# bioinf/Sibelia

Hardware: AMD Instinct MI355X
Metric: k-mers/sec in BlockFinder graph-build+simplify, 8xE.coli k=25 (higher is better)
Workload: dtype u64; 1 GPU; 8 synthetic E. coli-like strains x 4.6 Mbp (gen_strains seed 1, 1% SNP, indels, inversions), k=25 D=150 maxIterations=4, one full stage; strand_kmers_per_gpu=73598388, parallelism=1 GPU, exchange_bytes_rank0=0, bulges=334284, bif_ids=1120044, instances=7089276, rounds=106, replays=0, device_bytes=22762263122

## Files before the change

sibelia_amd/csrc/rounds.hip:

```cpp
#include <cstring>
#include <algorithm>
#include <vector>
#include "simplify_walks.h"

__device__ __forceinline__ int wave_probe_window(const GraphView &g, const ScanBurst &raw, unsigned dir, unsigned ws, VerdictTable &vt, unsigned lane,
                                                 unsigned id, unsigned tid, unsigned &distinct)
{
	ScanView b;
	burst_view(g, raw, dir, ws, lane, 3u, b);
	const unsigned k = g.k, D = g.D;
	if (k >= 64u * SCAN_BURST) return -2;
	unsigned firstbad = ~0u, firstsep = ~0u;
#pragma unroll
	for (int u = 0; u < SCAN_BURST; u++) {
		const unsigned long long in = __ballot(b.inr[u]), good = __ballot(b.inr[u] && b.plink[u] == b.cc[u]), sep = __ballot(b.inr[u] && b.chv[u] == BT_SEP);
		const unsigned long long bad = in & ~good;
		if (bad && firstbad == ~0u) firstbad = 64u * u + (unsigned)__builtin_ctzll(bad);
		if (sep && firstsep == ~0u) firstsep = 64u * u + (unsigned)__builtin_ctzll(sep);
	}
	const unsigned covered = ws < 64u * SCAN_BURST ? ws : 64u * SCAN_BURST;
	const unsigned len = firstsep < covered ? firstsep : covered;
	if (firstbad < len || firstbad <= firstsep && firstbad < covered) return -2;
	if (firstsep >= covered && covered < ws && D > covered) return -2;
	bool viol = false;
// ... 300 lines not shown
			const unsigned long long todo = __ballot(act && slow && j == 0u);
			if (pass == 1) {
				if (act && !slow) ecmask |= bit;
				for (unsigned long long td = todo; td; td &= td - 1ull) {
					const unsigned src = (unsigned)__builtin_ctzll(td);
					const unsigned wa = __shfl(a, src), wd = __shfl(dir, src);
					const WalkedWindow ww = idx_walk_window(g, wa, wd, k + 1u, lane, id, tid, nullptr, nullptr, 0u);
					if (ww.viol) viol = true;
					if (ww.len >= k + 1u) { const char e2 = wd ? bt_comp((char)ww.craw) : (char)ww.craw; ecmask |= e2 == 'A' ? 1u : e2 == 'C' ? 2u : e2 == 'G' ? 4u : 8u; }
				}
				continue;
			}
			const unsigned own = act ? s_own[i] : 0u;
			const unsigned lim = len < D ? len : D, upper = own < lim ? own : lim;
			unsigned long long cm = act && !slow && bit ? mk & vm & idx_bits(1 - t0, (int)upper - t0) : 0ull;
			unsigned total = (unsigned)__popcll(cm);
			for (int d = 32; d > 0; d >>= 1) total += __shfl_xor(total, d);
			const bool tight = distinct + total > VT_FILL;
			const unsigned *__restrict__ marks = g.bif[dir];
			while (__any(cm != 0ull)) {
				if (tight) {
					unsigned nins = (unsigned)__popcll(cm);
					nins = nins < 4u ? nins : 4u;
					for (int d = 32; d > 0; d >>= 1) nins += __shfl_xor(nins, d);
					if (distinct + nins > VT_HARD) return -1;
				}
				unsigned sl[4]; bool has[4]; unsigned bb[4];
#pragma unroll
				for (int q = 0; q < 4; q++) {
					has[q] = cm != 0ull;
					const unsigned r = has[q] ? (unsigned)__builtin_ctzll(cm) : 0u;
					if (has[q]) cm &= cm - 1ull;
					const unsigned step = (unsigned)(t0 + (int)r);
					sl[q] = has[q] ? (dir ? a - step : a + step) : a;
				}
#pragma unroll
				for (int q = 0; q < 4; q++) bb[q] = marks[fresh ? 0u : sl[q]];
				bool found = false;
#pragma unroll
				for (int q = 0; q < 4; q++) found |= vt_insert(vt, has[q] ? bb[q] : BT_NONE, bit, distinct);
				if (found) { if (viol) wave_stamp(g, 0, tid, 3, id, 0, tid + 1); return 1; }
			}
			for (unsigned long long td = todo; td; td &= td - 1ull) {
				const unsigned src = (unsigned)__builtin_ctzll(td);
				const unsigned wa = __shfl(a, src), wd = __shfl(dir, src);
				WSYNC();
				const WalkedWindow ww = idx_walk_window(g, wa, wd, ws, lane, id, tid, mk_step, mk_id, walk_marks);
				if (ww.viol) viol = true;
				if (ww.overflow) return -1;
				WSYNC();
				if (ww.len < k + 1u) continue;
				const char e2 = wd ? bt_comp((char)ww.craw) : (char)ww.craw;
				const unsigned b2 = e2 == 'A' ? 1u : e2 == 'C' ? 2u : e2 == 'G' ? 4u : 8u;
				const unsigned lim2 = ww.len < D ? ww.len : D;
				bool found = false;
				for (unsigned m0 = 0; m0 < ww.nm; m0 += 64) {
					if (distinct + (ww.nm - m0 < 64u ? ww.nm - m0 : 64u) > VT_HARD) return -1;
					const unsigned m = m0 + lane;
					const bool ok = m < ww.nm && mk_step[m] < lim2;
					found |= vt_insert(vt, ok ? mk_id[m] : BT_NONE, b2, distinct);
				}
				if (found) { if (viol) wave_stamp(g, 0, tid, 3, id, 0, tid + 1); return 1; }
			}
		}
		if (pass == 1) {
			for (int d = 32; d > 0; d >>= 1) ecmask |= __shfl_xor(ecmask, d);
			if (__popc(ecmask) <= 1) { if (viol) wave_stamp(g, 0, tid, 3, id, 0, tid + 1); return 0; }
		}
	}
	if (viol) wave_stamp(g, 0, tid, 3, id, 0, tid + 1);
	return 0;
}
__global__ void __launch_bounds__(64) k_probe_idx(GraphView g, unsigned nwin, uint8_t *live, unsigned w0, unsigned vbits, unsigned max_inst, unsigned walk_marks,
                                                  unsigned *__restrict__ instbuf, unsigned istride, int snapshot)
{
	extern __shared__ unsigned pidx_dyn[];
	VtRef vt; vt.key = pidx_dyn; vt.mask = pidx_dyn + (1u << vbits); vt.bits = vbits;
	unsigned *const s_sel = vt.mask + (1u << vbits), *const s_own = s_sel + max_inst, *const s_mkstep = s_own + max_inst, *const s_mkid = s_mkstep + walk_marks;
	uint8_t *const s_dir = reinterpret_cast<uint8_t *>(s_mkid + walk_marks);
	const unsigned wi = blockIdx.x + w0, lane = threadIdx.x;
	if (!snapshot) round_stamp(g, 0);
	if (wi >= nwin) return;
	const unsigned id = g.win[wi], tid = snapshot ? 0xFFFFFFFEu : id + 1;
	const bool known_live = !snapshot && g.need[id] == 2;
	if (known_live && !(instbuf && bt_parked(g, id))) { if (lane == 0) { live[wi] = 1; if (instbuf) instbuf[(size_t)wi * istride] = BT_NONE; if (g.test_flags & BT_TF_STATS) atomicAdd(&g_idx_stats[0], 1u); } return; }
	const unsigned n = wave_list_nodes(g, g.head[0][id], g.head[1][id], lane, nullptr, [&](unsigned off, unsigned, unsigned s, unsigned el, unsigned) {
		if (off < max_inst) { s_sel[off] = el; s_dir[off] = (uint8_t)s; }
	});
	int r = 0;
	if (known_live) {
		if (lane == 0) live[wi] = 1;
		unsigned *ib = instbuf + (size_t)wi * istride;
		const bool give = n <= max_inst && n + 1u <= istride;
		if (give) { WSYNC(); for (unsigned i = lane; i < n; i += 64) ib[1 + i] = (s_sel[i] << 1) | s_dir[i]; }
		if (lane == 0) ib[0] = give ? n : BT_NONE;
		return;
	}
	if (n >= 2) {
		if (n > max_inst || (!g.any_parked && n != g.lsize[0][id] + g.lsize[1][id])) r = -1;
		else { WSYNC(); r = probe_idx(g, vt, s_sel, s_dir, s_own, s_mkstep, s_mkid, walk_marks, n, lane, id, tid); }
	}
	if (lane == 0) {
		if (r < 0) live[wi] = PROBE_UNSERVED;
		else if (r == 0) { g.need[id] = 0; g.touch[id] = 0; live[wi] = 0; }
		else { g.need[id] = 2; live[wi] = 1; }
		if (g.test_flags & BT_TF_STATS) atomicAdd(&g_idx_stats[n < 2 ? 1 : r == 0 ? 2 : r == 1 ? 3 : r == -1 ? 4 : 5], 1u);
	}
	if (instbuf) {
		unsigned *ib = instbuf + (size_t)wi * istride;
		const bool give = r == 1 && n + 1u <= istride;
		if (give) { WSYNC(); for (unsigned i = lane; i < n; i += 64) ib[1 + i] = (s_sel[i] << 1) | s_dir[i]; }
		if (lane == 0) ib[0] = give ? n : BT_NONE;
	}
}

static_assert(PROBE_WAVES == 1u, "k_probe synchronises its lanes with WSYNC(): one wave per workgroup");
__global__ void __launch_bounds__(64 * PROBE_WAVES) k_probe(GraphView g, unsigned nwin, uint8_t *arena, unsigned arena_bytes, uint8_t *live, unsigned w0, int snapshot)
{
	__shared__ Txn t;
	__shared__ BulgeWork w;
	__shared__ VerdictTable vt;
	__shared__ int ok;
	__shared__ __attribute__((aligned(16))) uint8_t fast[2048];
	const unsigned wi = blockIdx.x + w0, lane = threadIdx.x & 63u;
	if (!g.idx_probe && !snapshot) round_stamp(g, 0);
	if (wi >= nwin) return;
	if ((g.idx_probe || snapshot) && live[wi] != PROBE_UNSERVED) return;
	const unsigned id = g.win[wi], tid = snapshot ? 0xFFFFFFFEu : id + 1;
	if (!snapshot && g.need[id] == 2) { if (threadIdx.x == 0) live[wi] = 1; return; }
	if (threadIdx.x == 0) { t.init(g, id, wi, snapshot ? 0u : 3u, arena + (size_t)(!snapshot && g.slice_busy && g.slice_busy[wi] ? g.shadow_base + wi : wi) * arena_bytes, arena_bytes); t.ext_stamps = true; t.fscr = fast; t.fscr_cap = sizeof fast; }
	WSYNC();
	wave_setup<true>(g, t, w, true, lane, ok);
	for (unsigned i = threadIdx.x; i < VT_SLOTS; i += 64 * PROBE_WAVES) { vt.key[i] = BT_NONE; vt.mask[i] = 0; }
	WSYNC();
	int verdict = 0;
	if (ok && probe_endchars(g, w, lane, id, tid)) ok = 0;
	if (ok) {
		verdict = probe_windows(g, w, vt, lane, id, tid);
		if (verdict < 0) {
			for (unsigned i = 0; i < w.n; i++) wave_scan_instance(g, w, i, lane, 0, tid, 3, id);
			WSYNC();
		}
	}
	if (lane == 0) {
		bool has = verdict > 0;
		if (verdict < 0) { bt_end_chars(t, w); has = bt_any_bulges(t, w, true); }
		if (t.err) has = true;
		if (!has) { g.need[id] = 0; g.touch[id] = 0; }
		else if (!t.err) g.need[id] = 2;
		else if (snapshot) g.need[id] = 1;
		live[wi] = has ? (t.err ? 2 : 1) : 0;
	}
}
__global__ void __launch_bounds__(256) k_pack_need(const unsigned *__restrict__ perm, const uint8_t *__restrict__ need, unsigned lo, unsigned hi, uint8_t *__restrict__ buf)
{
	const unsigned j = lo + blockIdx.x * blockDim.x + threadIdx.x;
	if (j < hi) buf[j] = need[perm[j]];
}
__global__ void __launch_bounds__(256) k_unpack_need(const unsigned *__restrict__ perm, const uint8_t *__restrict__ buf, unsigned n, unsigned mylo, unsigned myhi, uint8_t *__restrict__ need)
{
	const unsigned j = blockIdx.x * blockDim.x + threadIdx.x;
	if (j < n && (j < mylo || j >= myhi)) need[perm[j]] = buf[j];
}
__global__ void __launch_bounds__(256) k_pack_probe(const unsigned *__restrict__ ctr, const uint8_t *__restrict__ live, unsigned w0, unsigned w1, unsigned rank, unsigned stride, uint8_t *__restrict__ robuf)
{
	uint8_t *slot = robuf + (size_t)rank * stride;
	const unsigned i = blockIdx.x * blockDim.x + threadIdx.x;
	if (i == 0) *reinterpret_cast<unsigned *>(slot) = ctr[CTR_VIOL];
	if (w0 + i < w1) slot[4 + i] = live[w0 + i];
}
__global__ void __launch_bounds__(256) k_apply_probe(GraphView g, unsigned nwin, uint8_t *__restrict__ live, unsigned w0, unsigned w1, const uint8_t *__restrict__ robuf, unsigned stride, unsigned nranks)
{
	const unsigned wi = blockIdx.x * blockDim.x + threadIdx.x;
	if (wi == 0) { unsigned v = BT_NONE; for (unsigned p = 0; p < nranks; p++) { const unsigned t = *reinterpret_cast<const unsigned *>(robuf + (size_t)p * stride); v = t < v ? t : v; } if (v != BT_NONE) atomicMin(&g.ctr[CTR_VIOL], v); }
	if (wi >= nwin || (wi >= w0 && wi < w1)) return;
	unsigned p = (unsigned)(((unsigned long long)wi * nranks) / nwin);
	while ((unsigned)(((unsigned long long)nwin * p) / nranks) > wi) p--;
	while ((unsigned)(((unsigned long long)nwin * (p + 1)) / nranks) <= wi) p++;
	const uint8_t l = robuf[(size_t)p * stride + 4 + (wi - (unsigned)(((unsigned long long)nwin * p) / nranks))];
	live[wi] = l;
	const unsigned id = g.win[wi];
	if (l == 0) { g.need[id] = 0; g.touch[id] = 0; }
// ... 367 lines not shown
```

sibelia_amd/csrc/simplify.hip:

```cpp
#include <cstring>
#include <algorithm>
#include <array>
#include <chrono>

#include "sbl_ctx.h"
#include "sbl_prim.h"
#include "sbl_comm.h"
#include "kmer_kernels.h"
#include "simplify_driver.h"
#include "simplify_kernels.h"

static inline unsigned nblocks(size_t n, unsigned per) { return (unsigned)((n + per - 1) / per); }

struct SimplifyHandles {
	unsigned *h_ctr = nullptr;
	unsigned *d_hctr = nullptr;
	unsigned post_seq = 0;
	hipEvent_t ev[8] = {};
	std::vector<hipEvent_t> snap_ev;
	unsigned char *h_init = nullptr;
	~SimplifyHandles()
	{
		if (h_ctr) (void)hipHostFree(h_ctr);
		if (h_init) (void)hipHostFree(h_init);
// ... 187 lines not shown
		k_seg_tails<<<(ne + 255) / 256, 256, 0, s>>>(st->ch.as<uint8_t>(), st->nx.as<unsigned>(), ne, st->flag.as<unsigned>(), st->segidx.as<unsigned>(),
		                                            st->seg_head.as<unsigned>(), st->seg_len.as<unsigned>(), st->seg_succ_elem.as<unsigned>());
		k_seg_finish<<<(nseg + 255) / 256, 256, 0, s>>>(nseg, st->seg_head.as<unsigned>(), st->seg_len.as<unsigned>(), st->seg_succ_elem.as<unsigned>(),
		                                               st->flag.as<unsigned>(), st->segidx.as<unsigned>(), st->succ[0].as<unsigned>(), st->dist[0].as<unsigned long long>());
		int cur = 0;
		for (unsigned span = 1; span < nseg; span <<= 1, cur ^= 1)
			k_seg_jump<<<(nseg + 255) / 256, 256, 0, s>>>(nseg, st->succ[cur].as<unsigned>(), st->dist[cur].as<unsigned long long>(),
			                                             st->succ[cur ^ 1].as<unsigned>(), st->dist[cur ^ 1].as<unsigned long long>());
		unsigned long long total = 0;
		HIP_TRY(hipMemcpyAsync(&total, st->dist[cur].p, 8, hipMemcpyDeviceToHost, s));
		HIP_TRY(hipStreamSynchronize(s));
		*cur_out = cur;
		return total;
	}
	void linearise_marks(MarkStream &ms)
	{
		hipStream_t s = c->stream;
		const unsigned ne = ck_ne;
		int cur = 0;
		const unsigned long long total = rank_segments(ne, &cur);
		st->lin.ensure((size_t)ne * 4 + 16); st->elin.ensure((size_t)total * 4 + 16);
		k_lin_positions<<<(ne + 255) / 256, 256, 0, s>>>(st->ch.as<uint8_t>(), ne, st->flag.as<unsigned>(), st->segidx.as<unsigned>(), st->seg_head.as<unsigned>(),
		                                                st->dist[cur].as<unsigned long long>(), total, st->lin.as<unsigned>(), st->elin.as<unsigned>());
		const unsigned nchunks = (unsigned)((total + 1023) / 1024);
		st->cnt1k.ensure((size_t)(nchunks + 1) * 4); st->off1k.ensure((size_t)(nchunks + 1) * 4);
		for (int t = 0; t < 2; t++) {
			HIP_TRY(hipMemsetAsync(st->cnt1k.p, 0, (size_t)(nchunks + 1) * 4, s));
			k_count_marks_lin<<<nchunks, 256, 0, s>>>(c->d_bif[t].as<unsigned>(), st->elin.as<unsigned>(), (size_t)total, st->cnt1k.as<unsigned>());
			prim::exclusive_scan(s, st->scantmp, st->cnt1k.as<unsigned>(), st->off1k.as<unsigned>(), 0u, (size_t)nchunks + 1, rocprim::plus<unsigned>());
			unsigned nm = 0;
			HIP_TRY(hipMemcpyAsync(&nm, st->off1k.as<unsigned>() + nchunks, 4, hipMemcpyDeviceToHost, s));
			HIP_TRY(hipStreamSynchronize(s));
			st->lmpos[t].ensure((size_t)nm * 4 + 16); st->lmid[t].ensure((size_t)nm * 4 + 16); st->maux[t].ensure((size_t)nm * 4 + 16);
			if (nm) {
				k_write_marks_lin<<<nchunks, 256, 0, s>>>(c->d_bif[t].as<unsigned>(), st->elin.as<unsigned>(), st->nodeof[t].as<unsigned>(), (size_t)total, st->off1k.as<unsigned>(),
				                                         st->lmpos[t].as<unsigned>(), st->lmid[t].as<unsigned>(), st->nmark.as<unsigned>());
				k_mark_aux_lin<<<(nm + 255) / 256, 256, 0, s>>>(st->lmpos[t].as<unsigned>(), nm, (unsigned)t, c->d_sepidx.as<unsigned>(), c->nchr, st->lin.as<unsigned>(),
				                                               st->elin.as<unsigned>(), st->ch.as<uint8_t>(), g.k, st->maux[t].as<unsigned>());
			}
			ms.elem[t] = st->lmpos[t].as<unsigned>(); ms.id[t] = st->lmid[t].as<unsigned>(); ms.aux[t] = st->maux[t].as<unsigned>(); ms.n[t] = nm;
		}
		HIP_TRY(hipGetLastError());
	}
	bool few_touched()
	{
		unsigned *cnt = st->ctr.as<unsigned>() + CTR_TOUCHED, n = 0;
		HIP_TRY(hipMemsetAsync(cnt, 0, 4, c->stream));
		k_count_touched<<<256, 256, 0, c->stream>>>(st->touch.as<uint8_t>(), nid_, cnt);
		HIP_TRY(hipMemcpyAsync(&n, cnt, 4, hipMemcpyDeviceToHost, c->stream));
		HIP_TRY(hipStreamSynchronize(c->stream));
		return (unsigned long long)n * 16 < nid_ || n <= std::max<size_t>(1024, ne0_ >> 12);
	}
	bool split_ro() const { return c->comm && c->comm->n > 1 && !sw.replicated_phases; }
	double ro_ms = 0;
	void share(uint32_t n, uint32_t *lo, uint32_t *hi) const
	{
		const uint32_t R = c->comm->n, r = c->comm->rank;
		*lo = (uint32_t)((uint64_t)n * r / R); *hi = (uint32_t)((uint64_t)n * (r + 1) / R);
	}
	void allgather_shares(char *buf, uint32_t n, size_t es)
	{
		SblComm *cm = c->comm;
		const uint32_t R = cm->n, r = cm->rank;
		std::vector<size_t> sb(R), so(R), rb(R), ro(R);
		for (uint32_t p = 0; p < R; p++) {
			const size_t plo = (size_t)((uint64_t)n * p / R) * es, phi = (size_t)((uint64_t)n * (p + 1) / R) * es;
			const size_t mlo = (size_t)((uint64_t)n * r / R) * es, mhi = (size_t)((uint64_t)n * (r + 1) / R) * es;
			sb[p] = p == r ? 0 : mhi - mlo; so[p] = mlo;
			rb[p] = p == r ? 0 : phi - plo; ro[p] = plo;
			if (p != r) c->stats.verdict_bytes += mhi - mlo;
		}
		const auto t0 = std::chrono::steady_clock::now();
		try { cm->alltoallv(c, buf, sb.data(), so.data(), buf, rb.data(), ro.data()); }
		catch (...) { cm->abort_peers(); throw; }
		ro_ms += std::chrono::duration<double, std::milli>(std::chrono::steady_clock::now() - t0).count();
	}
	void allgather_slots(char *buf, uint32_t R, size_t es) { allgather_shares(buf, R, es); }
	uint32_t snap_slice = 0;
	void snapshot_idx()
	{
		unsigned *cnt = st->ctr.as<unsigned>() + CTR_TOUCHED, n = 0;
		st->snap_list.ensure((size_t)nid_ * 4 + 64); st->snap_live.ensure((size_t)nid_ + 64);
		HIP_TRY(hipMemsetAsync(cnt, 0, 4, c->stream));
		k_touched_list<<<(nid_ + 255) / 256, 256, 0, c->stream>>>(st->touch.as<uint8_t>(), nid_, st->snap_list.as<unsigned>(), cnt);
		HIP_TRY(hipMemcpyAsync(&n, cnt, 4, hipMemcpyDeviceToHost, c->stream));
		HIP_TRY(hipMemsetAsync(st->need.p, 0, (size_t)nid_ + 1, c->stream));
		HIP_TRY(hipMemsetAsync(st->touch.p, 0, (size_t)nid_ + 1, c->stream));
		HIP_TRY(hipStreamSynchronize(c->stream));
		const uint32_t slice = std::max<uint32_t>(1, snap_slice);
		for (uint32_t off = 0; off < n; off += slice) {
			const uint32_t m = std::min<uint32_t>(slice, n - off);
			GraphView gs = g;
			gs.win = st->snap_list.as<unsigned>() + off;
			gs.tstamp = nullptr;
			uint8_t *lv = st->snap_live.as<uint8_t>() + off;
			k_probe_idx<<<m, 64, pidx_lds(), c->stream>>>(gs, m, lv, 0u, pidx_vbits, pidx_inst, pidx_marks, nullptr, 0u, 1);
			k_probe<<<m, 64 * PROBE_WAVES, 0, c->stream>>>(gs, m, st->arena.as<uint8_t>(), arena_bytes, lv, 0u, 1);
		}
		HIP_TRY(hipGetLastError());
	}
	void snapshot_all(bool incremental)
	{
		while (st->snap_ev.size() < 2 * (size_t)(snap_used + 1)) { hipEvent_t e; HIP_TRY(hipEventCreate(&e)); st->snap_ev.push_back(e); }
		HIP_TRY(hipEventRecord(st->snap_ev[2 * snap_used], c->stream));
		uint32_t plo = 0, phi = nid_;
		const bool split = split_ro();
		if (split) share(nid_, &plo, &phi);
		if (!incremental) {
			MarkStream ms;
			for (int t = 0; t < 2; t++) { ms.elem[t] = c->d_melem[t].as<unsigned>(); ms.id[t] = c->d_mid[t].as<unsigned>(); ms.aux[t] = st->maux[t].as<unsigned>(); ms.n[t] = c->nmarks[t]; }
			HIP_TRY(hipMemsetAsync(st->touch.p, 0, (size_t)nid_ + 1, c->stream));
			k_snapshot_first<<<256 * 32, 64, 0, c->stream>>>(g, ms, st->nmark.as<unsigned>(), st->perm.as<unsigned>(), plo, phi);
		} else if (g.idx_probe && !split) {
			snapshot_idx();
		} else if (!few_touched()) {
			st->nmark.ensure((size_t)cap_n * 4);
			MarkStream ms;
			linearise_marks(ms);
			k_snapshot_stream<<<256 * 32, 64, 0, c->stream>>>(g, ms, st->nmark.as<unsigned>(), st->perm.as<unsigned>(), 1, plo, phi);
		} else {
			st->snap_arena.ensure((size_t)snap_threads * snap_arena_bytes);
			k_snapshot<<<snap_threads, 64, 0, c->stream>>>(g, st->snap_arena.as<uint8_t>(), snap_arena_bytes, 1, st->perm.as<unsigned>(), plo, phi);
		}
		HIP_TRY(hipGetLastError());
		if (split) {
			st->robuf.ensure((size_t)nid_ + 64);
			if (phi > plo) k_pack_need<<<(phi - plo + 255) / 256, 256, 0, c->stream>>>(st->perm.as<unsigned>(), st->need.as<uint8_t>(), plo, phi, st->robuf.as<uint8_t>());
			allgather_shares(st->robuf.as<char>(), nid_, 1);
			if (nid_) k_unpack_need<<<(nid_ + 255) / 256, 256, 0, c->stream>>>(st->perm.as<unsigned>(), st->robuf.as<uint8_t>(), nid_, plo, phi, st->need.as<uint8_t>());
			HIP_TRY(hipMemsetAsync(st->touch.p, 0, (size_t)nid_ + 1, c->stream));
			HIP_TRY(hipGetLastError());
		}
		HIP_TRY(hipEventRecord(st->snap_ev[2 * snap_used + 1], c->stream));
		snap_used++;
	}
	void snapshots_collect()
	{
		for (unsigned i = 0; i < snap_used; i++) {
			float ms = 0;
			HIP_TRY(hipEventSynchronize(st->snap_ev[2 * i + 1]));
			HIP_TRY(hipEventElapsedTime(&ms, st->snap_ev[2 * i], st->snap_ev[2 * i + 1]));
			snapshot_ms += ms;
		}
		snap_used = 0;
	}
	void park_sweep() { if (g.park_cap) k_park_sweep<<<nblocks((size_t)nid_ + 1, 256), 256, 0, c->stream>>>(st->park_of.as<unsigned>(), nid_ + 1); }
	void reset_round_state(bool stamps_too)
	{
		if (!stamps_too) park_sweep();
		if (stamps_too && g.park_cap) {
			HIP_TRY(hipMemsetAsync(st->park_of.p, 0, ((size_t)nid_ + 1) * 4, c->stream));
			HIP_TRY(hipMemsetAsync(st->slice_busy.p, 0, park_slices, c->stream));
			parked_known = 0; g.park_hold = 0;
		}
		HIP_TRY(hipMemsetAsync(st->own.p, 0xFF, ((size_t)nid_ + 1) * 4, c->stream));
		if (stamps_too) {
			HIP_TRY(hipMemsetAsync(st->rmax.p, 0, nres * 4, c->stream));
			HIP_TRY(hipMemsetAsync(st->wmax.p, 0, nres * 4, c->stream));
			if (g.bidx) k_idx_clear_stamps<<<(idx_nblk + 255) / 256, 256, 0, c->stream>>>(st->bidx.as<unsigned long long>(), idx_nblk);
		}
	}
	void clear_counters()
	{
		k_clear_counters<<<1, 256, 0, c->stream>>>(st->ctr.as<unsigned>());
		HIP_TRY(hipGetLastError());
	}
	bool sel_pending = false, sel_ready = false;
	uint32_t probed_nwin = 0;
	void select_launch(uint32_t lo, uint32_t limit, uint32_t W)
	{
		unsigned chunk = 8192;
		while ((unsigned long long)chunk * 1024 < (unsigned long long)nid_ + 1) chunk <<= 1;
		const unsigned chunk0 = lo / chunk, nchunks = limit / chunk - chunk0 + 1;
		GraphView gs = g;
		if (sel_stamped) gs.tslot = TS_CAP * 4;
		sel_stamped = true;
		k_select_count<<<nchunks, SEL_THREADS, 0, c->stream>>>(gs, st->sel.as<unsigned>(), lo, limit, chunk0, chunk, st->live.as<uint8_t>(), probed_nwin);
		probed_nwin = 0;
		posted = st->d_hctr != nullptr;
		if (posted) st->post_seq++;
		k_select_write<<<nchunks, SEL_THREADS, 0, c->stream>>>(g, st->sel.as<unsigned>(), st->win.as<unsigned>(), lo, limit, W, chunk0, chunk, nchunks, st->d_hctr, st->post_seq);
		HIP_TRY(hipGetLastError());
		sel_pending = true; sel_ready = false;
	}
	void select_read(uint32_t *nwin, uint32_t *newlo, uint32_t *solo)
	{
		if (!sel_ready) read_ctr();
		sel_pending = sel_ready = false;
		*nwin = st->h_ctr[CTR_NWIN]; *newlo = st->h_ctr[CTR_LO]; *solo = st->h_ctr[CTR_PUSHED];
		last_lo = *newlo;
	}
	enum { TS_CAP = 16384 };
	uint32_t ts_round = 0;
	bool sel_stamped = true;
	std::vector<uint8_t> ts_kind;
// ... 544 lines not shown
```

sibelia_amd/csrc/simplify_kernels.h:

```cpp
#pragma once
#include "sbl_ctx.h"
#include "simplify_steps.h"

#define CLAIM_CAP 4096u
#define PROBE_WAVES 1u
#define PROBE_UNSERVED 3u
#define SEL_THREADS 256
#define RSV_WAVES_MAX 4u
struct MarkStream { const unsigned *elem[2], *id[2], *aux[2]; unsigned n[2]; };

void sbl_commit_prof_reset();
void sbl_commit_prof_report(unsigned ts_round);
void sbl_rounds_stats_report();

__global__ void __launch_bounds__(256) k_init_links(unsigned *__restrict__ nx, unsigned *__restrict__ pv, unsigned *__restrict__ nodeof0,
                                                    unsigned *__restrict__ nodeof1, uint8_t *__restrict__ ch, size_t E, size_t cap);
__global__ void __launch_bounds__(256) k_instance_keys(const unsigned *__restrict__ elem, const unsigned *__restrict__ id, unsigned n, unsigned strand,
                                                       const unsigned *__restrict__ sepidx, unsigned nchr, unsigned E, unsigned ordbits,
                                                       unsigned long long *__restrict__ keys, unsigned *__restrict__ midx);
__global__ void __launch_bounds__(256) k_build_lists(const unsigned long long *__restrict__ skeys, const unsigned *__restrict__ smidx, const unsigned *__restrict__ melem, unsigned n,
                                                     unsigned node_base, unsigned strand, unsigned ordbits, unsigned *__restrict__ nslot, unsigned *__restrict__ nnext, unsigned *__restrict__ nidst,
                                                     uint8_t *__restrict__ ndead, unsigned *__restrict__ head, unsigned *__restrict__ lsize,
                                                     unsigned *__restrict__ nodeof, unsigned *__restrict__ nmark);
__global__ void __launch_bounds__(256) k_id_position_keys(const unsigned *__restrict__ head0, const unsigned *__restrict__ head1, const unsigned *__restrict__ nslot,
                                                          unsigned nid, unsigned long long *__restrict__ keys, unsigned *__restrict__ ids);
__global__ void __launch_bounds__(256) k_max_instances(const unsigned *__restrict__ l0, const unsigned *__restrict__ l1, unsigned nid, unsigned *__restrict__ out);
__global__ void __launch_bounds__(256) k_mark_aux(const unsigned *__restrict__ melem, unsigned n, unsigned strand, const unsigned *__restrict__ sepidx, unsigned nchr,
                                                  const uint8_t *__restrict__ ch, unsigned k, unsigned *__restrict__ aux);
__global__ void __launch_bounds__(64) k_snapshot_first(GraphView g, MarkStream ms, const unsigned *__restrict__ nmark, const unsigned *__restrict__ perm, unsigned plo, unsigned phi);
__global__ void __launch_bounds__(256) k_lin_positions(const uint8_t *__restrict__ ch, unsigned ne, const unsigned *__restrict__ flag, const unsigned *__restrict__ segidx,
                                                       const unsigned *__restrict__ seg_head, const unsigned long long *__restrict__ dist, unsigned long long total,
                                                       unsigned *__restrict__ lin, unsigned *__restrict__ elin);
__global__ void __launch_bounds__(256) k_count_marks_lin(const unsigned *__restrict__ bif, const unsigned *__restrict__ elin, size_t n, unsigned *__restrict__ chunkcnt);
__global__ void __launch_bounds__(256) k_write_marks_lin(const unsigned *__restrict__ bif, const unsigned *__restrict__ elin, const unsigned *__restrict__ nodeof, size_t n,
                                                         const unsigned *__restrict__ chunkoff, unsigned *__restrict__ out_pos, unsigned *__restrict__ out_id, unsigned *__restrict__ nmark);
__global__ void __launch_bounds__(256) k_mark_aux_lin(const unsigned *__restrict__ mpos, unsigned n, unsigned strand, const unsigned *__restrict__ sepelem, unsigned nchr,
                                                      const unsigned *__restrict__ lin, const unsigned *__restrict__ elin, const uint8_t *__restrict__ ch, unsigned k, unsigned *__restrict__ aux);
__global__ void __launch_bounds__(64) k_snapshot_stream(GraphView g, MarkStream ms, const unsigned *__restrict__ nmark, const unsigned *__restrict__ perm, int incremental, unsigned plo, unsigned phi);
__global__ void __launch_bounds__(64) k_snapshot(GraphView g, uint8_t *arena, unsigned arena_bytes, int incremental, const unsigned *__restrict__ perm, unsigned plo, unsigned phi);
__global__ void __launch_bounds__(64) k_probe_idx(GraphView g, unsigned nwin, uint8_t *live, unsigned w0, unsigned vbits, unsigned max_inst, unsigned walk_marks,
                                                  unsigned *__restrict__ instbuf, unsigned istride, int snapshot);
__global__ void __launch_bounds__(64 * PROBE_WAVES) k_probe(GraphView g, unsigned nwin, uint8_t *arena, unsigned arena_bytes, uint8_t *live, unsigned w0, int snapshot);
__global__ void __launch_bounds__(256) k_pack_need(const unsigned *__restrict__ perm, const uint8_t *__restrict__ need, unsigned lo, unsigned hi, uint8_t *__restrict__ buf);
__global__ void __launch_bounds__(256) k_unpack_need(const unsigned *__restrict__ perm, const uint8_t *__restrict__ buf, unsigned n, unsigned mylo, unsigned myhi, uint8_t *__restrict__ need);
__global__ void __launch_bounds__(256) k_apply_probe(GraphView g, unsigned nwin, uint8_t *__restrict__ live, unsigned w0, unsigned w1, const uint8_t *__restrict__ robuf, unsigned stride, unsigned nranks);
__global__ void __launch_bounds__(SEL_THREADS) k_select_count(GraphView g, unsigned *__restrict__ sel, unsigned lo, unsigned limit, unsigned chunk0, unsigned chunk,
                                                              const uint8_t *__restrict__ live, unsigned probed);
__global__ void __launch_bounds__(SEL_THREADS) k_select_write(GraphView g, unsigned *__restrict__ sel, unsigned *__restrict__ win, unsigned lo, unsigned limit, unsigned W,
                                                              unsigned chunk0, unsigned chunk, unsigned nchunks, volatile unsigned *post, unsigned post_seq);
__global__ void __launch_bounds__(256) k_pack_probe(const unsigned *__restrict__ ctr, const uint8_t *__restrict__ live, unsigned w0, unsigned w1, unsigned rank, unsigned stride, uint8_t *__restrict__ robuf);
__global__ void __launch_bounds__(64 * RSV_WAVES_MAX) k_reserve(GraphView g, unsigned nwin, unsigned *claims, const uint8_t *live, unsigned seen_bits, unsigned list_cap,
                                                                 const unsigned *__restrict__ instbuf, unsigned istride, const uint8_t *arena, unsigned arena_bytes);
__global__ void __launch_bounds__(64) __attribute__((amdgpu_waves_per_eu(4, 4))) k_commit(GraphView g, unsigned nwin, uint8_t *arena, unsigned arena_bytes, int solo, const unsigned *claims, const uint8_t *live, int prof);
__global__ void __launch_bounds__(256) k_park_sweep(unsigned *__restrict__ park_of, unsigned n);
__global__ void __launch_bounds__(64) k_chain(GraphView g, uint8_t *arena, unsigned arena_bytes, unsigned nwin, int prof);
__global__ void __launch_bounds__(64) k_dense_stage(GraphView g, uint8_t *arena, unsigned arena_bytes, unsigned max_iter, unsigned *out);
__global__ void __launch_bounds__(256) k_count_touched(const uint8_t *__restrict__ touch, unsigned nid, unsigned *__restrict__ out);
__global__ void __launch_bounds__(256) k_touched_list(const uint8_t *__restrict__ touch, unsigned nid, unsigned *__restrict__ list, unsigned *__restrict__ count);
__global__ void __launch_bounds__(256) k_seg_flags(const uint8_t *__restrict__ ch, const unsigned *__restrict__ nx, unsigned ne, unsigned *__restrict__ flag);
__global__ void __launch_bounds__(256) k_seg_tails(const uint8_t *__restrict__ ch, const unsigned *__restrict__ nx, unsigned ne,
                                                   const unsigned *__restrict__ flag, const unsigned *__restrict__ segidx ,
                                                   unsigned *__restrict__ seg_head, unsigned *__restrict__ seg_len, unsigned *__restrict__ seg_succ_elem);
__global__ void __launch_bounds__(256) k_seg_finish(unsigned nseg, const unsigned *__restrict__ seg_head, unsigned *__restrict__ seg_len,
                                                    const unsigned *__restrict__ seg_succ_elem, const unsigned *__restrict__ flag,
                                                    const unsigned *__restrict__ segidx, unsigned *__restrict__ succ, unsigned long long *__restrict__ dist);
__global__ void __launch_bounds__(256) k_seg_jump(unsigned nseg, const unsigned *__restrict__ succ_in, const unsigned long long *__restrict__ dist_in,
                                                  unsigned *__restrict__ succ_out, unsigned long long *__restrict__ dist_out);
__global__ void __launch_bounds__(256) k_scatter_linear(const uint8_t *__restrict__ ch, const unsigned *__restrict__ op, unsigned ne,
                                                        const unsigned *__restrict__ flag, const unsigned *__restrict__ segidx,
                                                        const unsigned *__restrict__ seg_head, const unsigned long long *__restrict__ dist,
                                                        unsigned long long total, uint8_t *__restrict__ ch_out, unsigned *__restrict__ op_out,
                                                        unsigned *__restrict__ newidx);
__global__ void k_remap_seps(const unsigned *__restrict__ newidx, unsigned *__restrict__ sepidx, unsigned n);
__global__ void k_sep_positions(const unsigned *__restrict__ sepidx, unsigned nchr, unsigned *__restrict__ op);
__global__ void __launch_bounds__(256) k_dict_check(const uint8_t *__restrict__ ch, unsigned ne, const unsigned *__restrict__ newidx, const uint8_t *__restrict__ ch_out, unsigned long long total,
                                                    const unsigned *__restrict__ bif0, const unsigned *__restrict__ bif1, const unsigned long long *__restrict__ dict, unsigned nd, unsigned k,
                                                    unsigned long long *__restrict__ out);
__global__ void __launch_bounds__(256) k_fill_bytes(uint8_t *p, uint8_t v, size_t from, size_t to);
__global__ void __launch_bounds__(256) k_build_blkidx(const uint8_t *__restrict__ ch, const unsigned *__restrict__ nx, const unsigned *__restrict__ pv,
                                                      const unsigned *__restrict__ bif0, const unsigned *__restrict__ bif1, unsigned norig, unsigned nblk,
                                                      unsigned long long *__restrict__ bidx);
__global__ void __launch_bounds__(256) k_check_blkidx(const uint8_t *__restrict__ ch, const unsigned *__restrict__ nx, const unsigned *__restrict__ pv,
                                                      const unsigned *__restrict__ bif0, const unsigned *__restrict__ bif1, const unsigned *__restrict__ wmax, unsigned norig, unsigned nblk,
                                                      const unsigned long long *__restrict__ bidx, unsigned *__restrict__ out);
__global__ void __launch_bounds__(256) k_clear_counters(unsigned *__restrict__ ctr);
__global__ void __launch_bounds__(256) k_idx_clear_stamps(unsigned long long *__restrict__ bidx, unsigned nblk);
```

sibelia_amd/csrc/snapshot.hip:

```cpp
#include <cstring>
#include <algorithm>
#include <vector>
#include "simplify_device.h"

__global__ void __launch_bounds__(256) k_mark_aux(const unsigned *__restrict__ melem, unsigned n, unsigned strand, const unsigned *__restrict__ sepidx, unsigned nchr,
                                                  const uint8_t *__restrict__ ch, unsigned k, unsigned *__restrict__ aux)
{
	unsigned i = blockIdx.x * blockDim.x + threadIdx.x;
	if (i >= n) return;
	const unsigned e = melem[i], c = chr_of(sepidx, nchr, e);
	const unsigned dist = strand == 0 ? sepidx[c + 1] - e : e - sepidx[c];
	unsigned bit = 0;
	if (dist >= k + 1) {
		const uint8_t x = strand == 0 ? ch[e + k] : ch[e - k];
		const unsigned code = x == 'A' ? 0u : x == 'C' ? 1u : x == 'G' ? 2u : 3u;
		bit = 1u << (strand == 0 ? code : 3u - code);
	}
	aux[i] = (bit << 24) | (dist < 0xFFFFFFu ? dist : 0xFFFFFFu);
}


__global__ void __launch_bounds__(64) k_snapshot_first(GraphView g, MarkStream ms, const unsigned *__restrict__ nmark, const unsigned *__restrict__ perm, unsigned plo, unsigned phi)
{
	__shared__ VerdictTable vt;
	const unsigned lane = threadIdx.x, sub = lane >> 4, sl = lane & 15u;
	const unsigned per = gridDim.x >> 3, slot = (blockIdx.x & 7u) * per + (blockIdx.x >> 3);
	for (unsigned base = plo; base < phi; base += gridDim.x) {
		if (base + slot >= phi) continue;
		const unsigned id = perm[base + slot];
		const unsigned n0 = g.lsize[0][id], n1 = g.lsize[1][id], n = n0 + n1;
		if (n < 2) { if (lane == 0) g.need[id] = 0; continue; }
		const unsigned h0 = g.head[0][id], h1 = g.head[1][id];
		{
			unsigned bits = 0;
			for (unsigned i = lane; i < n; i += 64) { const unsigned s = i >= n0 ? 1u : 0u, nd = s ? h1 + (i - n0) : h0 + i; bits |= ms.aux[s][nmark[nd]] >> 24; }
#pragma unroll
			for (int d = 32; d > 0; d >>= 1) bits |= __shfl_xor(bits, d);
			if (__popc(bits) <= 1) { if (lane == 0) g.need[id] = 0; continue; }
		}
		WSYNC();
		for (unsigned i = lane; i < VT_SLOTS; i += 64) { vt.key[i] = BT_NONE; vt.mask[i] = 0; }
		WSYNC();
		bool found = false, undecided = false;
		unsigned distinct = 0;
		for (unsigned ib = 0; ib < n && !found && !undecided; ib += 4) {
			const unsigned i = ib + sub;
			const bool act = i < n;
			const unsigned s = act && i >= n0 ? 1u : 0u;
			const unsigned nd = s ? h1 + (i - n0) : h0 + i;
			const unsigned j = act ? nmark[nd] : 0u;
			const unsigned ax = act ? ms.aux[s][j] : 0u, pos = act ? ms.elem[s][j] : 0u;
			const unsigned bit = ax >> 24, dist = ax & 0xFFFFFFu, lim = dist < g.D ? dist : g.D;
			bool go = act && bit != 0;
			for (unsigned t = 0; __any(go); t += 16) {
				const unsigned off = t + sl;
				const bool inr = go && (s == 0 ? (unsigned long long)j + 1 + off < ms.n[0] : off < j);
				const unsigned jj = s == 0 ? j + 1 + off : j - 1 - off;
				const unsigned p = inr ? ms.elem[s][jj] : 0u, b = inr ? ms.id[s][jj] : BT_NONE;
				const unsigned step = s == 0 ? p - pos : pos - p;
				const bool stop = !inr || step >= lim || b == id;
				const unsigned long long bal = __ballot(stop);
				const unsigned grp = (unsigned)(bal >> (sub * 16)) & 0xFFFFu;
				const unsigned upto = grp ? (unsigned)__builtin_ctz(grp) : 16u;
				const unsigned total = (unsigned)__popcll(__ballot(go && sl < upto));
				if (distinct + total > (VT_SLOTS * 3) / 4) { undecided = true; break; }
				bool fresh = false;
				if (go && sl < upto) {
					unsigned h = (b * 2654435761u) >> 23;
					for (;;) {
						unsigned old = atomicCAS(&vt.key[h], BT_NONE, b);
						if (old == BT_NONE || old == b) {
							fresh = old == BT_NONE;
							unsigned m = atomicOr(&vt.mask[h], bit) | bit;
							if (m & (m - 1)) found = true;
							break;
						}
						h = (h + 1) & (VT_SLOTS - 1);
					}
				}
				distinct += (unsigned)__popcll(__ballot(fresh));
				if (__any(found)) { found = true; break; }
				if (upto < 16) go = false;
			}
		}
		if (lane == 0) g.need[id] = found ? 2 : undecided ? 1 : 0;
	}
}

__global__ void __launch_bounds__(256) k_lin_positions(const uint8_t *__restrict__ ch, unsigned ne, const unsigned *__restrict__ flag, const unsigned *__restrict__ segidx,
                                                       const unsigned *__restrict__ seg_head, const unsigned long long *__restrict__ dist, unsigned long long total,
                                                       unsigned *__restrict__ lin, unsigned *__restrict__ elin)
{
	unsigned e = blockIdx.x * blockDim.x + threadIdx.x;
	if (e >= ne) return;
	if (ch[e] == BT_DEAD_CHAR) { lin[e] = SBL_NONE; return; }
	unsigned seg = segidx[e] + flag[e] - 1;
	unsigned pos = (unsigned)(total - dist[seg] + (e - seg_head[seg]));
	lin[e] = pos; elin[pos] = e;
}
__global__ void __launch_bounds__(256) k_count_marks_lin(const unsigned *__restrict__ bif, const unsigned *__restrict__ elin, size_t n, unsigned *__restrict__ chunkcnt)
{
	__shared__ unsigned cnt;
	if (threadIdx.x == 0) cnt = 0;
	__syncthreads();
	size_t base = (size_t)blockIdx.x * 1024;
	unsigned c = 0;
	for (unsigned i = threadIdx.x; i < 1024; i += 256) { size_t p = base + i; c += (p < n && bif[elin[p]] != SBL_NONE); }
	atomicAdd(&cnt, c);
	__syncthreads();
	if (threadIdx.x == 0) chunkcnt[blockIdx.x] = cnt;
}
__global__ void __launch_bounds__(256) k_write_marks_lin(const unsigned *__restrict__ bif, const unsigned *__restrict__ elin, const unsigned *__restrict__ nodeof, size_t n,
// ... 67 lines not shown
			const bool act = i < n;
			const unsigned packed = act ? s_inst[i] : 0u, s = packed & 1u, j = packed >> 1;
			const unsigned ax = act ? ms.aux[s][j] : 0u, pos = act ? ms.elem[s][j] : 0u;
			const unsigned bit = ax >> 24, dist = ax & 0xFFFFFFu, lim = dist < g.D ? dist : g.D;
			bool go = act && bit != 0;
			for (unsigned t = 0; __any(go); t += 16) {
				const unsigned off = t + sl;
				const bool inr = go && (s == 0 ? (unsigned long long)j + 1 + off < ms.n[0] : off < j);
				const unsigned jj = s == 0 ? j + 1 + off : j - 1 - off;
				const unsigned p = inr ? ms.elem[s][jj] : 0u, b = inr ? ms.id[s][jj] : BT_NONE;
				const unsigned step = s == 0 ? p - pos : pos - p;
				const bool stop = !inr || step >= lim || b == id;
				const unsigned long long bal = __ballot(stop);
				const unsigned grp = (unsigned)(bal >> (sub * 16)) & 0xFFFFu;
				const unsigned upto = grp ? (unsigned)__builtin_ctz(grp) : 16u;
				const unsigned total = (unsigned)__popcll(__ballot(go && sl < upto));
				if (distinct + total > (VT_SLOTS * 3) / 4) { undecided = true; break; }
				bool fresh = false;
				if (go && sl < upto) {
					unsigned h = (b * 2654435761u) >> 23;
					for (;;) {
						unsigned old = atomicCAS(&vt.key[h], BT_NONE, b);
						if (old == BT_NONE || old == b) {
							fresh = old == BT_NONE;
							unsigned m = atomicOr(&vt.mask[h], bit) | bit;
							if (m & (m - 1)) found = true;
							break;
						}
						h = (h + 1) & (VT_SLOTS - 1);
					}
				}
				distinct += (unsigned)__popcll(__ballot(fresh));
				if (__any(found)) { found = true; break; }
				if (upto < 16) go = false;
			}
		}
		if (lane == 0) g.need[id] = found ? 2 : undecided ? 1 : 0;
	}
}

__global__ void __launch_bounds__(64) k_snapshot(GraphView g, uint8_t *arena, unsigned arena_bytes, int incremental, const unsigned *__restrict__ perm, unsigned plo, unsigned phi)
{
	__shared__ Txn t;
	__shared__ BulgeWork w;
	__shared__ VerdictTable vt;
	__shared__ int ok;
	__shared__ __attribute__((aligned(16))) uint8_t fast[2048];
	const unsigned lane = threadIdx.x;
	uint8_t *mine = arena + (size_t)blockIdx.x * arena_bytes;
	const unsigned per = gridDim.x >> 3, slot = (blockIdx.x & 7u) * per + (blockIdx.x >> 3);
	for (unsigned base = plo; base < phi; base += gridDim.x) {
		if (base + slot >= phi) continue;
		const unsigned id = perm[base + slot];
		if (incremental && !g.touch[id]) { if (lane == 0) g.need[id] = 0; continue; }
		WSYNC();
		if (lane == 0) { g.touch[id] = 0; t.init(g, id, 0, 0, mine, arena_bytes); t.fscr = fast; t.fscr_cap = sizeof fast; }
		WSYNC();
		wave_setup(g, t, w, true, lane, ok);
		if (ok) {
			wave_scan_all(g, w, lane, 0, 0, 0, id);
			WSYNC();
		}
		int verdict = ok ? wave_verdict(g, w, vt, lane) : 0;
		if (lane == 0) {
			bool v = verdict > 0;
			if (verdict < 0) { bt_end_chars(t, w); v = bt_any_bulges(t, w, true); }
			if (t.err & BT_ERR_SCRATCH) v = true;
			g.need[id] = v ? (verdict > 0 ? 2 : 1) : 0;
		}
	}
}

__global__ void __launch_bounds__(256) k_count_touched(const uint8_t *__restrict__ touch, unsigned nid, unsigned *__restrict__ out)
{
	unsigned c = 0;
	for (unsigned i = blockIdx.x * blockDim.x + threadIdx.x; i < nid; i += gridDim.x * blockDim.x) c += touch[i] != 0;
#pragma unroll
	for (int d = 32; d > 0; d >>= 1) c += __shfl_down(c, d);
	if ((threadIdx.x & 63) == 0 && c) atomicAdd(out, c);
}

__global__ void __launch_bounds__(256) k_touched_list(const uint8_t *__restrict__ touch, unsigned nid, unsigned *__restrict__ list, unsigned *__restrict__ count)
{
	const unsigned id = blockIdx.x * blockDim.x + threadIdx.x, lane = threadIdx.x & 63u;
	const bool t = id < nid && touch[id] != 0;
	const unsigned long long m = __ballot(t);
	if (!m) return;
	unsigned base = 0;
	if (lane == (unsigned)__builtin_ctzll(m)) base = atomicAdd(count, (unsigned)__popcll(m));
	base = __shfl(base, (unsigned)__builtin_ctzll(m));
	if (t) list[base + (unsigned)__popcll(m & ((1ull << lane) - 1ull))] = id;
}
```

Measured before the change: 1.372 billion strand-k-mers/s.

## Prefilter snapshot candidates into a compacted list and vectorise touched-list scan

Adds a thread-per-id prefilter kernel that checks up to 16 instances' aux bits and writes only ids needing a full wave-level check into a compacted list, so k_snapshot_first no longer spends a 64-lane wave on every id in the range. k_touched_list now reads 16 touch bytes per thread with a uint4 load and does one atomic per block via a wave scan and LDS. k_probe_idx hoists need, head, lsize and park lookups into registers at the start. The cost is an extra kernel launch and a list write, and the output list order is now nondeterministic.

```diff
diff --git a/sibelia_amd/csrc/rounds.hip b/sibelia_amd/csrc/rounds.hip
--- a/sibelia_amd/csrc/rounds.hip
+++ b/sibelia_amd/csrc/rounds.hip
@@ -406,9 +406,12 @@
 	if (!snapshot) round_stamp(g, 0);
 	if (wi >= nwin) return;
 	const unsigned id = g.win[wi], tid = snapshot ? 0xFFFFFFFEu : id + 1;
-	const bool known_live = !snapshot && g.need[id] == 2;
-	if (known_live && !(instbuf && bt_parked(g, id))) { if (lane == 0) { live[wi] = 1; if (instbuf) instbuf[(size_t)wi * istride] = BT_NONE; if (g.test_flags & BT_TF_STATS) atomicAdd(&g_idx_stats[0], 1u); } return; }
-	const unsigned n = wave_list_nodes(g, g.head[0][id], g.head[1][id], lane, nullptr, [&](unsigned off, unsigned, unsigned s, unsigned el, unsigned) {
+	const unsigned need = g.need[id], h0 = g.head[0][id], h1 = g.head[1][id], lsz = g.lsize[0][id] + g.lsize[1][id];
+	const unsigned pk = g.park_of ? g.park_of[id] : 0u;
+	const bool parked = pk != 0 && !(pk >> 31);
+	const bool known_live = !snapshot && need == 2;
+	if (known_live && !(instbuf && parked)) { if (lane == 0) { live[wi] = 1; if (instbuf) instbuf[(size_t)wi * istride] = BT_NONE; if (g.test_flags & BT_TF_STATS) atomicAdd(&g_idx_stats[0], 1u); } return; }
+	const unsigned n = wave_list_nodes(g, h0, h1, lane, nullptr, [&](unsigned off, unsigned, unsigned s, unsigned el, unsigned) {
 		if (off < max_inst) { s_sel[off] = el; s_dir[off] = (uint8_t)s; }
 	});
 	int r = 0;
@@ -421,7 +424,7 @@
 		return;
 	}
 	if (n >= 2) {
-		if (n > max_inst || (!g.any_parked && n != g.lsize[0][id] + g.lsize[1][id])) r = -1;
+		if (n > max_inst || (!g.any_parked && n != lsz)) r = -1;
 		else { WSYNC(); r = probe_idx(g, vt, s_sel, s_dir, s_own, s_mkstep, s_mkid, walk_marks, n, lane, id, tid); }
 	}
 	if (lane == 0) {
diff --git a/sibelia_amd/csrc/simplify.hip b/sibelia_amd/csrc/simplify.hip
--- a/sibelia_amd/csrc/simplify.hip
+++ b/sibelia_amd/csrc/simplify.hip
@@ -293,7 +293,7 @@
 		unsigned *cnt = st->ctr.as<unsigned>() + CTR_TOUCHED, n = 0;
 		st->snap_list.ensure((size_t)nid_ * 4 + 64); st->snap_live.ensure((size_t)nid_ + 64);
 		HIP_TRY(hipMemsetAsync(cnt, 0, 4, c->stream));
-		k_touched_list<<<(nid_ + 255) / 256, 256, 0, c->stream>>>(st->touch.as<uint8_t>(), nid_, st->snap_list.as<unsigned>(), cnt);
+		k_touched_list<<<(nid_ + 256 * TOUCH_PER_THREAD - 1) / (256 * TOUCH_PER_THREAD), 256, 0, c->stream>>>(st->touch.as<uint8_t>(), nid_, st->snap_list.as<unsigned>(), cnt);
 		HIP_TRY(hipMemcpyAsync(&n, cnt, 4, hipMemcpyDeviceToHost, c->stream));
 		HIP_TRY(hipMemsetAsync(st->need.p, 0, (size_t)nid_ + 1, c->stream));
 		HIP_TRY(hipMemsetAsync(st->touch.p, 0, (size_t)nid_ + 1, c->stream));
@@ -321,7 +321,13 @@
 			MarkStream ms;
 			for (int t = 0; t < 2; t++) { ms.elem[t] = c->d_melem[t].as<unsigned>(); ms.id[t] = c->d_mid[t].as<unsigned>(); ms.aux[t] = st->maux[t].as<unsigned>(); ms.n[t] = c->nmarks[t]; }
 			HIP_TRY(hipMemsetAsync(st->touch.p, 0, (size_t)nid_ + 1, c->stream));
-			k_snapshot_first<<<256 * 32, 64, 0, c->stream>>>(g, ms, st->nmark.as<unsigned>(), st->perm.as<unsigned>(), plo, phi);
+			unsigned *cnt = st->ctr.as<unsigned>() + CTR_TOUCHED;
+			st->snap_list.ensure((size_t)nid_ * 4 + 64);
+			HIP_TRY(hipMemsetAsync(cnt, 0, 4, c->stream));
+			if (phi > plo) {
+				k_snapshot_prefilter<<<(phi - plo + 255) / 256, 256, 0, c->stream>>>(g, ms, st->nmark.as<unsigned>(), st->perm.as<unsigned>(), plo, phi, st->snap_list.as<unsigned>(), cnt);
+				k_snapshot_first<<<256 * 32, 64, 0, c->stream>>>(g, ms, st->nmark.as<unsigned>(), st->snap_list.as<unsigned>(), cnt);
+			}
 		} else if (g.idx_probe && !split) {
 			snapshot_idx();
 		} else if (!few_touched()) {
diff --git a/sibelia_amd/csrc/simplify_kernels.h b/sibelia_amd/csrc/simplify_kernels.h
--- a/sibelia_amd/csrc/simplify_kernels.h
+++ b/sibelia_amd/csrc/simplify_kernels.h
@@ -27,7 +27,9 @@
 __global__ void __launch_bounds__(256) k_max_instances(const unsigned *__restrict__ l0, const unsigned *__restrict__ l1, unsigned nid, unsigned *__restrict__ out);
 __global__ void __launch_bounds__(256) k_mark_aux(const unsigned *__restrict__ melem, unsigned n, unsigned strand, const unsigned *__restrict__ sepidx, unsigned nchr,
                                                   const uint8_t *__restrict__ ch, unsigned k, unsigned *__restrict__ aux);
-__global__ void __launch_bounds__(64) k_snapshot_first(GraphView g, MarkStream ms, const unsigned *__restrict__ nmark, const unsigned *__restrict__ perm, unsigned plo, unsigned phi);
+__global__ void __launch_bounds__(256) k_snapshot_prefilter(GraphView g, MarkStream ms, const unsigned *__restrict__ nmark, const unsigned *__restrict__ perm, unsigned plo, unsigned phi,
+                                                            unsigned *__restrict__ list, unsigned *__restrict__ count);
+__global__ void __launch_bounds__(64) k_snapshot_first(GraphView g, MarkStream ms, const unsigned *__restrict__ nmark, const unsigned *__restrict__ list, const unsigned *__restrict__ count);
 __global__ void __launch_bounds__(256) k_lin_positions(const uint8_t *__restrict__ ch, unsigned ne, const unsigned *__restrict__ flag, const unsigned *__restrict__ segidx,
                                                        const unsigned *__restrict__ seg_head, const unsigned long long *__restrict__ dist, unsigned long long total,
                                                        unsigned *__restrict__ lin, unsigned *__restrict__ elin);
@@ -56,6 +58,7 @@
 __global__ void __launch_bounds__(64) k_chain(GraphView g, uint8_t *arena, unsigned arena_bytes, unsigned nwin, int prof);
 __global__ void __launch_bounds__(64) k_dense_stage(GraphView g, uint8_t *arena, unsigned arena_bytes, unsigned max_iter, unsigned *out);
 __global__ void __launch_bounds__(256) k_count_touched(const uint8_t *__restrict__ touch, unsigned nid, unsigned *__restrict__ out);
+#define TOUCH_PER_THREAD 16u
 __global__ void __launch_bounds__(256) k_touched_list(const uint8_t *__restrict__ touch, unsigned nid, unsigned *__restrict__ list, unsigned *__restrict__ count);
 __global__ void __launch_bounds__(256) k_seg_flags(const uint8_t *__restrict__ ch, const unsigned *__restrict__ nx, unsigned ne, unsigned *__restrict__ flag);
 __global__ void __launch_bounds__(256) k_seg_tails(const uint8_t *__restrict__ ch, const unsigned *__restrict__ nx, unsigned ne,
diff --git a/sibelia_amd/csrc/snapshot.hip b/sibelia_amd/csrc/snapshot.hip
--- a/sibelia_amd/csrc/snapshot.hip
+++ b/sibelia_amd/csrc/snapshot.hip
@@ -20,14 +20,55 @@
 }
 
 
-__global__ void __launch_bounds__(64) k_snapshot_first(GraphView g, MarkStream ms, const unsigned *__restrict__ nmark, const unsigned *__restrict__ perm, unsigned plo, unsigned phi)
+#define SNAP_PRE_INST 16u
+__global__ void __launch_bounds__(256) k_snapshot_prefilter(GraphView g, MarkStream ms, const unsigned *__restrict__ nmark, const unsigned *__restrict__ perm, unsigned plo, unsigned phi,
+                                                            unsigned *__restrict__ list, unsigned *__restrict__ count)
+{
+	__shared__ unsigned s_wave[4], s_base;
+	const unsigned lane = threadIdx.x & 63u, wv = threadIdx.x >> 6;
+	const unsigned long long p = (unsigned long long)plo + blockIdx.x * 256u + threadIdx.x;
+	const bool act = p < phi;
+	const unsigned id = act ? perm[p] : 0u;
+	bool keep = false;
+	if (act) {
+		const unsigned n0 = g.lsize[0][id], n1 = g.lsize[1][id], h0 = g.head[0][id], h1 = g.head[1][id], n = n0 + n1;
+		if (n >= 2) {
+			const unsigned *__restrict__ a0 = ms.aux[0], *__restrict__ a1 = ms.aux[1];
+			const unsigned m = n < SNAP_PRE_INST ? n : SNAP_PRE_INST;
+			unsigned bits = 0;
+			for (unsigned i0 = 0; i0 < m && __popc(bits) <= 1; i0 += 4) {
+				unsigned j[4], ax[4];
+#pragma unroll
+				for (int q = 0; q < 4; q++) { const unsigned i = i0 + q; j[q] = i < m ? nmark[i >= n0 ? h1 + (i - n0) : h0 + i] : 0u; }
+#pragma unroll
+				for (int q = 0; q < 4; q++) { const unsigned i = i0 + q; ax[q] = i < m ? (i >= n0 ? a1 : a0)[j[q]] : 0u; }
+#pragma unroll
+				for (int q = 0; q < 4; q++) bits |= ax[q] >> 24;
+			}
+			keep = __popc(bits) > 1 || n > m;
+		}
+		if (!keep) g.need[id] = 0;
+	}
+	const unsigned long long km = __ballot(keep);
+	if (lane == 0) s_wave[wv] = (unsigned)__popcll(km);
+	__syncthreads();
+	if (threadIdx.x == 0) { const unsigned total = s_wave[0] + s_wave[1] + s_wave[2] + s_wave[3]; s_base = total ? atomicAdd(count, total) : 0u; }
+	__syncthreads();
+	if (keep) {
+		unsigned off = s_base + (unsigned)__popcll(km & ((1ull << lane) - 1ull));
+		for (unsigned x = 0; x < wv; x++) off += s_wave[x];
+		list[off] = id;
+	}
+}
+__global__ void __launch_bounds__(64) k_snapshot_first(GraphView g, MarkStream ms, const unsigned *__restrict__ nmark, const unsigned *__restrict__ list, const unsigned *__restrict__ count)
 {
 	__shared__ VerdictTable vt;
 	const unsigned lane = threadIdx.x, sub = lane >> 4, sl = lane & 15u;
 	const unsigned per = gridDim.x >> 3, slot = (blockIdx.x & 7u) * per + (blockIdx.x >> 3);
-	for (unsigned base = plo; base < phi; base += gridDim.x) {
+	const unsigned phi = *count;
+	for (unsigned base = 0; base < phi; base += gridDim.x) {
 		if (base + slot >= phi) continue;
-		const unsigned id = perm[base + slot];
+		const unsigned id = list[base + slot];
 		const unsigned n0 = g.lsize[0][id], n1 = g.lsize[1][id], n = n0 + n1;
 		if (n < 2) { if (lane == 0) g.need[id] = 0; continue; }
 		const unsigned h0 = g.head[0][id], h1 = g.head[1][id];
@@ -261,12 +302,27 @@
 
 __global__ void __launch_bounds__(256) k_touched_list(const uint8_t *__restrict__ touch, unsigned nid, unsigned *__restrict__ list, unsigned *__restrict__ count)
 {
-	const unsigned id = blockIdx.x * blockDim.x + threadIdx.x, lane = threadIdx.x & 63u;
-	const bool t = id < nid && touch[id] != 0;
-	const unsigned long long m = __ballot(t);
-	if (!m) return;
-	unsigned base = 0;
-	if (lane == (unsigned)__builtin_ctzll(m)) base = atomicAdd(count, (unsigned)__popcll(m));
-	base = __shfl(base, (unsigned)__builtin_ctzll(m));
-	if (t) list[base + (unsigned)__popcll(m & ((1ull << lane) - 1ull))] = id;
-}
+	__shared__ unsigned s_wave[4], s_base;
+	const unsigned lane = threadIdx.x & 63u, wv = threadIdx.x >> 6;
+	const unsigned long long id0 = ((unsigned long long)blockIdx.x * 256u + threadIdx.x) * TOUCH_PER_THREAD;
+	unsigned m = 0;
+	if (id0 + TOUCH_PER_THREAD <= nid) {
+		const uint4 v = *reinterpret_cast<const uint4 *>(touch + id0);
+		const unsigned x[4] = { v.x, v.y, v.z, v.w };
+#pragma unroll
+		for (int j = 0; j < 16; j++) m |= ((x[j >> 2] >> (8 * (j & 3))) & 0xFFu) ? 1u << j : 0u;
+	} else {
+		for (unsigned j = 0; j < TOUCH_PER_THREAD; j++) if (id0 + j < nid && touch[id0 + j]) m |= 1u << j;
+	}
+	const unsigned cnt = (unsigned)__popc(m);
+	unsigned incl = cnt;
+#pragma unroll
+	for (int d = 1; d < 64; d <<= 1) { const unsigned v = __shfl_up(incl, d); if (lane >= (unsigned)d) incl += v; }
+	if (lane == 63) s_wave[wv] = incl;
+	__syncthreads();
+	if (threadIdx.x == 0) { const unsigned total = s_wave[0] + s_wave[1] + s_wave[2] + s_wave[3]; s_base = total ? atomicAdd(count, total) : 0u; }
+	__syncthreads();
+	unsigned off = s_base + incl - cnt;
+	for (unsigned x = 0; x < wv; x++) off += s_wave[x];
+	for (; m; m &= m - 1u) list[off++] = (unsigned)id0 + (unsigned)__builtin_ctz(m);
+}
```

New measurement: 1.385 billion strand-k-mers/s (median of 6 runs). Within noise of the previous version (+1.0%).
